# cschin/Peregrine

Measured on AMD Instinct MI355X. Metric: confirmed overlaps/sec (ovlp_t records, index+overlap stages, seqdb resident in HBM), higher is better.
Workload: dtype u8/u32 integer

## Files before the change

### peregrine_amd/csrc/pgx_align.hip

```cpp
#include <hipcub/hipcub.hpp>

#include "pgx_internal.h"

namespace pgx {
namespace {

__device__ __forceinline__ uint64_t load_u64_unaligned(const uint8_t *p) {
  uint64_t v;
  __builtin_memcpy(&v, p, 8);
  return v;
}
struct U128 {
  uint64_t lo, hi;
};
__device__ __forceinline__ U128 load_u128_unaligned(const uint8_t *p) {
  U128 v;
  __builtin_memcpy(&v, p, 16);
  return v;
}
__device__ __forceinline__ int match8(uint64_t qa, uint64_t ta, int qs, int ts) {
  const uint64_t diff = ((qa >> qs) ^ (ta >> ts)) & 0x0F0F0F0F0F0F0F0FULL;
  return diff ? (__builtin_ctzll(diff) >> 3) : 8;
}
__device__ __forceinline__ uint64_t ballot64(bool p) { return __builtin_amdgcn_ballot_w64(p); }
template <int CTRL>
__device__ __forceinline__ int dpp_max(int v) {
  return max(v, __builtin_amdgcn_update_dpp(0, v, CTRL, 0xf, 0xf, true));
}
template <int GL>
__device__ __forceinline__ int group_max_i32(int v) {
  v = dpp_max<0xB1>(v);
  v = dpp_max<0x4E>(v);
  if (GL >= 8) v = dpp_max<0x141>(v);
  if (GL == 16) v = dpp_max<0x140>(v);
  return v;
}
template <int GL>
__device__ __forceinline__ uint32_t group_bits(uint64_t wave_mask, int gbase) {
  return (uint32_t)(wave_mask >> gbase) & ((1u << GL) - 1u);
}
template <int CTRL>
__device__ __forceinline__ int dpp_min(int v) {
  return min(v, __builtin_amdgcn_update_dpp(0, v, CTRL, 0xf, 0xf, true));
}
__device__ __forceinline__ int group_min8_i32(int v) {
  v = dpp_min<0xB1>(v);
  v = dpp_min<0x4E>(v);
  return dpp_min<0x141>(v);
}
__device__ __forceinline__ uint32_t ffbl_or_ones(uint32_t v) {
  uint32_t r;
  asm("v_ffbl_b32 %0, %1" : "=v"(r) : "v"(v));
  return r;
}
__device__ __forceinline__ int group_lane(int v, int gb4, int l) { return __builtin_amdgcn_ds_bpermute(gb4 + (l << 2), v); }

template <int CTRL, int ROW_MASK>
__device__ __forceinline__ int dpp_max_step(int v) {
  return max(v, __builtin_amdgcn_update_dpp(v, v, CTRL, ROW_MASK, 0xf, false));
}
__device__ __forceinline__ int wave_max_i32(int v) {
  v = dpp_max_step<0x111, 0xf>(v);
  v = dpp_max_step<0x112, 0xf>(v);
  v = dpp_max_step<0x114, 0xf>(v);
  v = dpp_max_step<0x118, 0xf>(v);
  v = dpp_max_step<0x142, 0xa>(v);
  v = dpp_max_step<0x143, 0xc>(v);
  return __builtin_amdgcn_readlane(v, 63);
}


}

__device__ __forceinline__ int match16p(const uint8_t *q, uint32_t xq, const uint8_t *t, uint32_t yt) {
  uint2 qd, td;
  __builtin_memcpy(&qd, q + (xq >> 4) * 4, 8), __builtin_memcpy(&td, t + (yt >> 4) * 4, 8);
  const uint32_t df = __builtin_amdgcn_alignbit(qd.y, qd.x, (xq & 15) << 1) ^ __builtin_amdgcn_alignbit(td.y, td.x, (yt & 15) << 1);
  return (int)min(ffbl_or_ones(df) >> 1, 16u);
}
template <bool PACKED>
__device__ __forceinline__ void align_one_per_wave(const uint8_t *__restrict__ seq, const uint64_t *__restrict__ roff,
                                                   const uint32_t *__restrict__ rlen, const pgx_align_key *__restrict__ keys, uint32_t a, int band,
                                                   int ring, pgx_match *__restrict__ out) {
  extern __shared__ int32_t V[];
  constexpr int PB = PACKED ? 16 : 8;
  const int lane = threadIdx.x;
  const pgx_align_key key = keys[a];
  const uint32_t len0 = rlen[key.rid0], len1 = rlen[key.rid1];
  const uint8_t *q = PACKED ? seq + (roff[key.rid0] + (key.dir0 ? (len0 + 15u) >> 4 : 0u) + (key.q_off >> 4)) * 4 : seq + roff[key.rid0] + key.q_off;
  const uint8_t *t = PACKED ? seq + (roff[key.rid1] + (key.dir1 ? (len1 + 15u) >> 4 : 0u)) * 4 : seq + roff[key.rid1];
  const uint32_t qo = PACKED ? key.q_off & 15u : 0u;
  const int q_len = (int)(len0 - key.q_off);
  const int t_len = (int)len1;
  const int qs = key.dir0 ? 4 : 0, ts = key.dir1 ? 4 : 0;
  const int max_d = (int)(0.3 * (double)(q_len + t_len));
  const int band_size = band * 2;
  const int mask = ring - 1;
  for (int i = lane; i < ring; i += 64) V[i] = 0;
  __syncthreads();

  int best_m = -1, min_k = 0, max_k = 0;
  uint32_t longest = 0;
  bool started = false, matched = false;
  int q_bgn = 0, t_bgn = 0, q_m_end = 0, t_m_end = 0, q_end = 0, t_end = 0, dist = 0;

  for (int d = 0; d < max_d; ++d) {
    if (max_k - min_k > band_size) break;
    const int nk = max_k >= min_k ? ((max_k - min_k) >> 1) + 1 : 0;
    int x = 0, y = 0;
    for (int base = 0; base < nk && !matched; base += 64) {
      const int j = base + lane;
      const bool active = j < nk;
      const int k = min_k + 2 * j;
      int x1 = 0, y1 = 0;
      x = 0, y = 0;
      bool more = false;
      if (active) {
        const int va = V[(k - 1) & mask], vb = V[(k + 1) & mask];
        x = (k == min_k || (k != max_k && va < vb)) ? vb : va + 1;
        y = x - k;
        x1 = x, y1 = y;
        const int rem = min(q_len - x, t_len - y);
        if (rem > 0) {
          int m = PACKED ? match16p(q, qo + (uint32_t)x, t, (uint32_t)y) : match8(load_u64_unaligned(q + x), load_u64_unaligned(t + y), qs, ts);
          m = min(m, rem);
          x += m, y += m;
          more = (m == PB) && (rem > PB);
        }
      }
      uint64_t mm = ballot64(more);
      while (mm) {
        const int L = __builtin_ctzll(mm);
        const int xs = __builtin_amdgcn_readlane(x, L), ys = __builtin_amdgcn_readlane(y, L);
        const int rem = min(q_len - xs, t_len - ys);
        const int off = lane * PB;
        int m = 0;
        if (off < rem)
          m = min(PACKED ? match16p(q, qo + (uint32_t)(xs + off), t, (uint32_t)(ys + off))
                         : match8(load_u64_unaligned(q + xs + off), load_u64_unaligned(t + ys + off), qs, ts), rem - off);
        const uint64_t stop = ballot64(m < PB);
        int ext;
        if (stop) {
          const int f = __builtin_ctzll(stop);
          ext = PB * f + __builtin_amdgcn_readlane(m, f);
        } else {
          ext = 64 * PB;
        }
        if (lane == L) x += ext, y += ext;
        if (stop || ext >= rem) mm &= mm - 1;
      }
      const int ext = x - x1;
      const bool hit = active && (x >= q_len || y >= t_len);
      const uint64_t hitmask = ballot64(hit);
      const int hl = hitmask ? __builtin_ctzll(hitmask) : 64;
      const bool valid = active && lane <= hl;
      if (!started) {
        const uint64_t m = ballot64(valid && ext > 16);
        if (m) {
          const int l = __builtin_ctzll(m);
          q_bgn = __builtin_amdgcn_readlane(x1, l), t_bgn = __builtin_amdgcn_readlane(y1, l);
          started = true;
        }
      }
      if (ballot64(valid && (uint32_t)ext > longest)) {
        const int mx = wave_max_i32(valid ? ext : -1);
        const int l = __builtin_ctzll(ballot64(valid && ext == mx));
        longest = (uint32_t)mx;
        q_m_end = __builtin_amdgcn_readlane(x, l), t_m_end = __builtin_amdgcn_readlane(y, l);
      }
      if (valid) V[k & mask] = x;
      best_m = max(best_m, wave_max_i32(valid ? x + y : -1));
      if (hitmask) {
        matched = true;
        q_end = __builtin_amdgcn_readlane(x, hl), t_end = __builtin_amdgcn_readlane(y, hl);
      }
    }
    __syncthreads();
    if (matched) {
      dist = d;
      break;
    }
    int new_min = max_k, new_max = min_k;
    const int thr = best_m - band;
    for (int base = 0; base < nk; base += 64) {
      const int j = base + lane;
      const int k2 = min_k + 2 * j;
      int u;
      if (nk <= 64) u = x + y;
      else u = j < nk ? 2 * V[k2 & mask] - k2 : 0;
      const uint64_t m = ballot64(j < nk && u >= thr);
      if (m) {
        new_min = min(new_min, min_k + 2 * (base + __builtin_ctzll(m)));
        new_max = max(new_max, min_k + 2 * (base + 63 - __builtin_clzll(m)));
      }
    }
    max_k = new_max + 1;
    min_k = new_min - 1;
  }
  if (lane == 0) {
    pgx_match r;
    if (matched) {
      r.q_bgn = q_bgn, r.t_bgn = t_bgn, r.q_end = q_end, r.t_end = t_end, r.dist = dist;
      r.m_size = (q_end - q_bgn + t_end - t_bgn + 2 * dist) / 2;
    } else {
      r.q_bgn = 0, r.t_bgn = 0, r.q_end = 0, r.t_end = 0, r.dist = 0, r.m_size = 0;
    }
    r.q_m_end = q_m_end, r.t_m_end = t_m_end;
    out[a] = r;
  }
}
template <bool PACKED>
__global__ __launch_bounds__(64) void k_align1(const uint8_t *__restrict__ seq, const uint64_t *__restrict__ roff,
                                              const uint32_t *__restrict__ rlen,
                                              const pgx_align_key *__restrict__ keys, uint32_t n, int band,
                                              int ring, pgx_match *__restrict__ out) {
  if (blockIdx.x < n) align_one_per_wave<PACKED>(seq, roff, rlen, keys, blockIdx.x, band, ring, out);
}
template <bool PACKED>
__global__ __launch_bounds__(64) void k_align1_list(const uint8_t *__restrict__ seq, const uint64_t *__restrict__ roff,
                                                   const uint32_t *__restrict__ rlen, const pgx_align_key *__restrict__ keys,
                                                   const uint32_t *__restrict__ list_n, const uint32_t *__restrict__ list, int band, int ring,
                                                   pgx_match *__restrict__ out) {
  const uint32_t cnt = *list_n;
  for (uint32_t i = blockIdx.x; i < cnt; i += gridDim.x) {
    __syncthreads();
    align_one_per_wave<PACKED>(seq, roff, rlen, keys, list[i], band, ring, out);
  }
}


template <int GL, typename VT>
__global__ __launch_bounds__(64) void k_align4(const uint8_t *__restrict__ seq, const uint64_t *__restrict__ roff,
                                               const uint32_t *__restrict__ rlen,
                                               const pgx_align_key *__restrict__ keys, uint32_t n, int band, int ring,
                                               pgx_match *__restrict__ out, uint32_t *__restrict__ counter) {
  extern __shared__ int32_t Vall[];
  const int lane = threadIdx.x, gl = lane & (GL - 1), gbase = lane & ~(GL - 1);
  VT *V = reinterpret_cast<VT *>(Vall) + (lane / GL) * ring;
  const int mask = ring - 1, band_size = band * 2;

  uint32_t c_next = 0, c_end = 0;
  bool alive = false, exhausted = false;
  uint32_t a = 0;
  const uint8_t *q = seq, *t = seq;
  int q_len = 0, t_len = 0, qs = 0, ts = 0, max_d = 0, d = 0;
  int best_m = -1, min_k = 0, max_k = 0;
  uint32_t longest = 0;
  bool started = false, matched = false;
  int q_bgn = 0, t_bgn = 0, q_m_end = 0, t_m_end = 0, q_end = 0, t_end = 0;

  for (;;) {
    const bool fetching = !alive && !exhausted;
    const uint64_t fw = ballot64(fetching);
    uint32_t na = 0;
    if (fw) {
      constexpr uint32_t CHUNK = 8;
      uint64_t need = 0;
      for (int g = 0; g < 64; g += GL) need |= 1ULL << g;
      need &= fw;
      const uint32_t cnt = (uint32_t)__builtin_popcountll(need);
      const uint32_t r = __builtin_amdgcn_mbcnt_hi((uint32_t)(need >> 32), __builtin_amdgcn_mbcnt_lo((uint32_t)need, 0u));
      const uint32_t avail = __builtin_amdgcn_readfirstlane(c_end - c_next);
      na = c_next + r;
      if (avail < cnt) {
        uint32_t got = 0;
        if (lane == 0) got = atomicAdd(counter, CHUNK);
        got = __builtin_amdgcn_readfirstlane(got);
        if (r >= avail) na = got + (r - avail);
        c_next = got + (cnt - avail), c_end = got + CHUNK;
      } else {
        c_next += cnt;
      }
    }
    if (fetching) {
      na = (uint32_t)__shfl((int)na, gbase, 64);
      if (na >= n) {
        exhausted = true;
      } else {
        a = na;
        const pgx_align_key key = keys[a];
        q = seq + roff[key.rid0] + key.q_off;
        t = seq + roff[key.rid1];
        q_len = (int)(rlen[key.rid0] - key.q_off);
        t_len = (int)rlen[key.rid1];
        qs = key.dir0 ? 4 : 0, ts = key.dir1 ? 4 : 0;
        max_d = (int)(0.3 * (double)(q_len + t_len));
        d = 0, best_m = -1, min_k = 0, max_k = 0, longest = 0;
        started = matched = false;
        q_bgn = t_bgn = q_m_end = t_m_end = q_end = t_end = 0;
        if (gl == 0) V[1 & mask] = (VT)0;
        alive = true;
      }
    }
    if (!ballot64(alive)) break;
    __syncthreads();

    bool stepping = alive;
    if (alive && (d >= max_d || max_k - min_k > band_size)) {
      if (gl == 0) {
        pgx_match r;
        r.m_size = 0, r.dist = 0, r.q_bgn = 0, r.q_end = 0, r.t_bgn = 0, r.t_end = 0;
        r.t_m_end = t_m_end, r.q_m_end = q_m_end;
        out[a] = r;
      }
      alive = false, stepping = false;
    }

    const int nk = max_k >= min_k ? ((max_k - min_k) >> 1) + 1 : 0;
    int x = 0, y = 0;
    for (int base = 0;; base += GL) {
      const bool inround = stepping && !matched && base < nk;
      if (!ballot64(inround)) break;
      const int j = base + gl;
      const bool active = inround && j < nk;
      const int k = min_k + 2 * j;
      int x1 = 0, y1 = 0;
      bool more = false;
      if (inround) x = 0, y = 0;
      if (active) {
        const int va = (int)V[(k - 1) & mask], vb = (int)V[(k + 1) & mask];
        x = (k == min_k || (k != max_k && va < vb)) ? vb : va + 1;
        y = x - k;
        x1 = x, y1 = y;
        const int rem = min(q_len - x, t_len - y);
        if (rem > 0) {
          int m = match8(load_u64_unaligned(q + x), load_u64_unaligned(t + y), qs, ts);
          m = min(m, rem);
          x += m, y += m;
          more = (m == 8) && (rem > 8);
        }
      }
      uint64_t mw = ballot64(more);
      while (mw) {
        const uint32_t gm = group_bits<GL>(mw, gbase);
        const bool has = gm != 0;
        const int L = has ? __builtin_ctz(gm) : 0;
        const int xs = __shfl(x, gbase + L, 64), ys = __shfl(y, gbase + L, 64);
        const int rem = min(q_len - xs, t_len - ys);
        constexpr int SL = GL == 16 ? 8 : 16;
        const int off = gl * SL;
        int m = SL;
        if (has) {
          m = 0;
          if (off < rem) {
            m = match8(load_u64_unaligned(q + xs + off), load_u64_unaligned(t + ys + off), qs, ts);
            if (SL == 16 && m == 8 && off + 8 < rem)
              m += match8(load_u64_unaligned(q + xs + off + 8), load_u64_unaligned(t + ys + off + 8), qs, ts);
            m = min(m, rem - off);
          }
        }
        const uint32_t sg = group_bits<GL>(ballot64(has && m < SL), gbase);
        int ext = GL * SL;
        if (sg) {
          const int f = __builtin_ctz(sg);
          ext = SL * f + __shfl(m, gbase + f, 64);
        }
        if (has && gl == L) {
          x += ext, y += ext;
          if (sg || ext >= rem) more = false;
        }
        mw = ballot64(more);
      }
      const int ext = x - x1;
      const bool hit = active && (x >= q_len || y >= t_len);
      const uint64_t hitw = ballot64(hit);
      int hl = GL;
      if (hitw) {
        const uint32_t hitm = group_bits<GL>(hitw, gbase);
        if (hitm) hl = __builtin_ctz(hitm);
      }
      const bool valid = active && gl <= hl;
      {
        const uint64_t sw = ballot64(valid && ext > 16 && !started);
        if (sw) {
          const uint32_t m = group_bits<GL>(sw, gbase);
          const int l = m ? __builtin_ctz(m) : 0;
          const int bx = __shfl(x1, gbase + l, 64), by = __shfl(y1, gbase + l, 64);
          if (m) q_bgn = bx, t_bgn = by, started = true;
        }
      }
      if (ballot64(valid && (uint32_t)ext > longest)) {
        const int mx = group_max_i32<GL>(valid ? ext : -1);
        const uint32_t m = group_bits<GL>(ballot64(valid && ext == mx), gbase);
        const int l = m ? __builtin_ctz(m) : 0;
        const int ex = __shfl(x, gbase + l, 64), ey = __shfl(y, gbase + l, 64);
        if (inround && mx >= 0 && (uint32_t)mx > longest) longest = (uint32_t)mx, q_m_end = ex, t_m_end = ey;
      }
      if (valid) V[k & mask] = (VT)x;
      {
        const int s = group_max_i32<GL>(valid ? x + y : -1);
        if (inround) best_m = max(best_m, s);
      }
      if (hitw) {
        const uint32_t hitm = group_bits<GL>(hitw, gbase);
        const int ex = __shfl(x, gbase + (hl & (GL - 1)), 64), ey = __shfl(y, gbase + (hl & (GL - 1)), 64);
        if (inround && hitm) matched = true, q_end = ex, t_end = ey;
      }
    }
    __syncthreads();

    if (stepping && matched) {
      if (gl == 0) {
        pgx_match r;
        r.q_bgn = q_bgn, r.t_bgn = t_bgn, r.q_end = q_end, r.t_end = t_end, r.dist = d;
        r.m_size = (q_end - q_bgn + t_end - t_bgn + 2 * d) / 2;
        r.t_m_end = t_m_end, r.q_m_end = q_m_end;
        out[a] = r;
      }
      alive = false, stepping = false;
    }
    int new_min = max_k, new_max = min_k;
    const int thr = best_m - band;
    for (int base = 0;; base += GL) {
      const bool inround = stepping && base < nk;
      if (!ballot64(inround)) break;
      const int j = base + gl;
      const int k2 = min_k + 2 * j;
      int u = 0;
      if (inround && j < nk) u = (nk <= GL) ? x + y : 2 * (int)V[k2 & mask] - k2;
      const uint32_t m = group_bits<GL>(ballot64(inround && j < nk && u >= thr), gbase);
      if (m) {
        new_min = min(new_min, min_k + 2 * (base + __builtin_ctz(m)));
        new_max = max(new_max, min_k + 2 * (base + 31 - __builtin_clz(m)));
      }
    }
    if (stepping) max_k = new_max + 1, min_k = new_min - 1, ++d;
  }
}


enum { PH_FETCH = 0, PH_STEP = 1, PH_ROUND = 2, PH_SNAKE = 3, PH_END = 4, PH_BAND = 5, PH_DONE = 6 };
#ifdef PGX_PH_BARRIER
#define PH_SYNC() __syncthreads()
#else
#define PH_SYNC() __builtin_amdgcn_fence(__ATOMIC_RELEASE, "wavefront"), __builtin_amdgcn_fence(__ATOMIC_ACQUIRE, "wavefront")
#endif
template <int GL, typename VT, bool PACKED>
__global__ __launch_bounds__(1024, 8) void k_align_ph(const uint8_t *__restrict__ seq, const uint64_t *__restrict__ roff,
                                                      const uint32_t *__restrict__ rlen, const pgx_align_key *__restrict__ keys,
                                                      uint32_t n, int band, int ring, pgx_match *__restrict__ out,
                                                      uint32_t *__restrict__ counter, const uint32_t *__restrict__ redo_n,
                                                      const uint32_t *__restrict__ redo_list, uint32_t *__restrict__ esc_n,
                                                      uint32_t *__restrict__ esc_list, const uint32_t *__restrict__ nflag, uint32_t seg,
                                                      uint32_t iter_limit) {
  extern __shared__ int32_t Vall[];
  __shared__ unsigned long long s_state;
  __shared__ uint32_t s_lock;
  static_assert(GL == 8, "the group operations below are written for 8-lane groups (half a DPP row)");
  const int lane = threadIdx.x & 63, gl = lane & (GL - 1), gbase = lane & ~(GL - 1), gb4 = gbase << 2;
  VT *V = reinterpret_cast<VT *>(Vall) + ((threadIdx.x >> 6) * (64 / GL) + lane / GL) * ring;
  if (threadIdx.x == 0) s_state = (unsigned long long)seg, s_lock = 0u;
  __syncthreads();
  const int mask = ring - 1, band_size = band * 2;
  constexpr int SL = PACKED ? 32 : (GL == 16 ? 8 : 16);
  constexpr int PROBE = PACKED ? 16 : 8;
  if (redo_list) n = *redo_n;
  const uint32_t iter_budget = esc_list && iter_limit ? iter_limit : 0xFFFFFFFFu;
  uint32_t qo = 0, to = 0;
  uint32_t iters = 0;
  uint32_t c_next = 0, c_end = 0;

  int phase = PH_FETCH;
  uint32_t a = 0;
  const uint8_t *q = seq, *t = seq;
  int q_len = 0, t_len = 0, qs = 0, ts = 0, max_d = 0, d = 0;
  int best_m = -1, min_k = 0, max_k = 0, nk = 0, base = 0, bbase = 0, new_min = 0, new_max = 0;
  uint32_t longest = 0;
  bool started = false;
  int q_bgn = 0, t_bgn = 0, q_m_end = 0, t_m_end = 0;
  int x = 0, y = 0, x1 = 0, y1 = 0, k = 0;
  bool active = false;
  uint32_t gm = 0;

#ifdef PGX_ALIGN_STATS
  uint32_t my_iters = 0;
  int my_maxnk = 0;
  bool has_cand = false;
#endif
  for (;;) {
#ifdef PGX_ALIGN_STATS
    if (phase == PH_FETCH && has_cand && gl == 0 && !redo_list) {
      const uint32_t b = my_iters ? 31u - (uint32_t)__builtin_clz(my_iters) : 0u;
      atomicAdd(counter + 1 + min(b, 31u), 1u);
#ifdef PGX_ALIGN_STATS_NK
      atomicAdd(counter + 33 + min((uint32_t)my_maxnk, 31u), 1u);
#else
      atomicAdd(counter + 33 + min(b, 31u), my_iters);
#endif
    }
    if (phase == PH_FETCH) has_cand = false, my_iters = 0, my_maxnk = 0;
    my_maxnk = max(my_maxnk, phase == PH_ROUND || phase == PH_STEP ? nk : 0);
    ++my_iters;
#endif
    ++iters;
    constexpr uint32_t RETRY = 0xFFFFFFFFu;
    const bool fetching = phase == PH_FETCH;
    const uint64_t fw = ballot64(fetching);
    uint32_t na = 0;
    if (fw) {
      constexpr uint32_t CHUNK = 8;
      const uint64_t need = fw & 0x0101010101010101ULL;
      const uint32_t cnt = (uint32_t)__builtin_popcountll(need);
      const uint32_t r = __builtin_amdgcn_mbcnt_hi((uint32_t)(need >> 32), __builtin_amdgcn_mbcnt_lo((uint32_t)need, 0u));
      const uint32_t avail = __builtin_amdgcn_readfirstlane(c_end - c_next);
      na = c_next + r;
      if (avail < cnt) {
        uint32_t got = RETRY;
        if (lane == 0) {
          unsigned long long o = atomicAdd(&s_state, (unsigned long long)CHUNK);
          if ((uint32_t)o < seg) {
            got = (uint32_t)(o >> 32) + (uint32_t)o;
          } else if (atomicCAS(&s_lock, 0u, 1u) == 0u) {
            o = atomicAdd(&s_state, (unsigned long long)CHUNK);
            if ((uint32_t)o < seg) {
              got = (uint32_t)(o >> 32) + (uint32_t)o;
            } else {
              got = atomicAdd(counter, seg);
              atomicExch(&s_state, ((unsigned long long)got << 32) | CHUNK);
            }
            atomicExch(&s_lock, 0u);
          }
        }
        got = __builtin_amdgcn_readfirstlane(got);
        if (got == RETRY) {
          if (r >= avail) na = RETRY;
          c_next = c_end = 0;
        } else {
          if (r >= avail) na = got + (r - avail);
          c_next = got + (cnt - avail), c_end = got + CHUNK;
        }
      } else {
        c_next += cnt;
      }
    }
    if (fetching) {
      iters = 0;
      na = (uint32_t)group_lane((int)na, gb4, 0);
      if (na == RETRY) {
      } else if (na >= n) {
        phase = PH_DONE;
      } else {
#ifdef PGX_ALIGN_STATS
        has_cand = true;
#endif
        a = redo_list ? redo_list[na] : na;
        const pgx_align_key key = keys[a];
        const uint32_t len0 = rlen[key.rid0], len1 = rlen[key.rid1];
        if (PACKED) {
          q = seq + (roff[key.rid0] + (key.dir0 ? (len0 + 15u) >> 4 : 0u) + (key.q_off >> 4)) * 4;
          t = seq + (roff[key.rid1] + (key.dir1 ? (len1 + 15u) >> 4 : 0u)) * 4;
          qo = key.q_off & 15u, to = 0;
        } else {
          q = seq + roff[key.rid0] + key.q_off;
          t = seq + roff[key.rid1];
        }
        q_len = (int)(len0 - key.q_off);
        t_len = (int)len1;
        qs = key.dir0 ? 4 : 0, ts = key.dir1 ? 4 : 0;
        max_d = (int)(0.3 * (double)(q_len + t_len));
        d = 0, best_m = -1, min_k = 0, max_k = 0, longest = 0;
        started = false;
        q_bgn = t_bgn = q_m_end = t_m_end = 0;
        if (gl == 0) V[1 & mask] = (VT)0;
        phase = PH_STEP;
        if (PACKED && ((nflag[key.rid0] | nflag[key.rid1]) & 1u)) {
          if (gl == 0) esc_list[n + atomicAdd(esc_n + 1, 1u)] = a;
          phase = PH_FETCH;
        }
      }
    }
    if (!ballot64(phase != PH_DONE)) break;
    PH_SYNC();

    if (iters > iter_budget && phase == PH_STEP && !(d >= max_d || max_k - min_k > band_size)) {
      if (gl == 0) esc_list[atomicAdd(esc_n, 1u)] = a;
      phase = PH_FETCH;
    }
    if (phase == PH_STEP) {
      const int width = max_k - min_k;
      if (d >= max_d || width > band_size) {
        if (gl == 0) {
          pgx_match r;
          r.m_size = 0, r.dist = 0, r.q_bgn = 0, r.q_end = 0, r.t_bgn = 0, r.t_end = 0;
          r.t_m_end = t_m_end, r.q_m_end = q_m_end;
          out[a] = r;
        }
        phase = PH_FETCH;
      } else if (width < 0) {
        nk = 0, base = 0, bbase = 0, new_min = max_k, new_max = min_k, phase = PH_BAND;
      } else {
        nk = (width >> 1) + 1, base = 0, phase = PH_ROUND;
      }
    }

    int probe_full = 0;
    if (phase == PH_ROUND) {
      const int j = base + gl;
      active = j < nk;
      k = min_k + 2 * j;
      if (active) {
        const int va = (int)V[(k - 1) & mask], vb = (int)V[(k + 1) & mask];
        x = (k == min_k || (k != max_k && va < vb)) ? vb : va + 1;
        y = x - k;
        x1 = x, y1 = y;
        const int rem = min(q_len - x, t_len - y);
        if (rem > 0) {
          int m;
          if (PACKED) {
            const uint32_t xq = qo + (uint32_t)x, yt = to + (uint32_t)y;
            uint2 qd, td;
            __builtin_memcpy(&qd, q + (xq >> 4) * 4, 8), __builtin_memcpy(&td, t + (yt >> 4) * 4, 8);
            const uint32_t df = __builtin_amdgcn_alignbit(qd.y, qd.x, (xq & 15) << 1) ^ __builtin_amdgcn_alignbit(td.y, td.x, (yt & 15) << 1);
            m = (int)min(ffbl_or_ones(df) >> 1, 16u);
          } else {
            m = match8(load_u64_unaligned(q + x), load_u64_unaligned(t + y), qs, ts);
          }
          probe_full = (int)min((uint32_t)m, (uint32_t)(rem - 1));
          m = (int)min((uint32_t)m, (uint32_t)rem);
          x += m, y += m;
        }
      }
    }
    {
      asm volatile("" : "+v"(probe_full));
      const uint32_t g = group_bits<GL>(ballot64(probe_full >= PROBE), gbase);
      if (phase == PH_ROUND) gm = g, phase = g ? PH_SNAKE : PH_END;
    }

    {
      const bool sn = phase == PH_SNAKE;
      if (ballot64(sn)) {
        const int L = __builtin_ctz(gm | 0x100u);
        const int xs = group_lane(x, gb4, L), ys = group_lane(y, gb4, L);
        const int rem = min(q_len - xs, t_len - ys);
        const int off = gl * SL;
        int e = GL * SL;
        if (sn) {
          e = off;
          if (off < rem) {
            int m;
            if (PACKED) {
              const uint32_t xq = qo + (uint32_t)(xs + off), yt = to + (uint32_t)(ys + off);
              uint4 qd, td;
              __builtin_memcpy(&qd, q + (xq >> 4) * 4, 16), __builtin_memcpy(&td, t + (yt >> 4) * 4, 16);
              const uint32_t qsh = (xq & 15) << 1, tsh = (yt & 15) << 1;
              const uint32_t d0 = __builtin_amdgcn_alignbit(qd.y, qd.x, qsh) ^ __builtin_amdgcn_alignbit(td.y, td.x, tsh);
              const uint32_t d1 = __builtin_amdgcn_alignbit(qd.z, qd.y, qsh) ^ __builtin_amdgcn_alignbit(td.z, td.y, tsh);
              m = (int)min(min(ffbl_or_ones(d0), ffbl_or_ones(d1) | 32u) >> 1, 32u);
            } else {
              const U128 qa = load_u128_unaligned(q + xs + off), ta = load_u128_unaligned(t + ys + off);
              m = match8(qa.lo, ta.lo, qs, ts);
              if (m == 8) m += match8(qa.hi, ta.hi, qs, ts);
            }
            m = (int)min((uint32_t)m, (uint32_t)(rem - off));
            e = m < SL ? off + m : GL * SL;
          }
        }
        const int ext = group_min8_i32(e);
        if (sn) {
          if (gl == L) x += ext, y += ext;
          if (ext < GL * SL || ext >= rem) gm &= gm - 1;
          if (!gm) phase = PH_END;
        }
      }
    }

    {
      const bool e = phase == PH_END;
      const int ext = x - x1;
      const bool hit = e && active && (x >= q_len || y >= t_len);
      const uint64_t hitw = ballot64(hit);
      int hl = GL;
      uint32_t hitm = 0;
      if (hitw) {
        hitm = group_bits<GL>(hitw, gbase);
        if (hitm) hl = __builtin_ctz(hitm);
        asm volatile("" : "+v"(hl));
      }
      const bool valid = e && active && gl <= hl;
      {
        const uint64_t sw = ballot64((valid && !started ? ext : 0) > 16);
        if (sw) {
          const uint32_t m = group_bits<GL>(sw, gbase);
          const int l = m ? __builtin_ctz(m) : 0;
          const int bx = group_lane(x1, gb4, l), by = group_lane(y1, gb4, l);
          if (m) q_bgn = bx, t_bgn = by, started = true;
        }
      }
      const int ev = valid ? ext : -1;
      if (ballot64(ev > (int)longest)) {
        const int mx = group_max_i32<GL>(ev);
        const uint32_t m = group_bits<GL>(ballot64(valid && ext == mx), gbase);
        const int l = m ? __builtin_ctz(m) : 0;
        const int ex = group_lane(x, gb4, l), ey = group_lane(y, gb4, l);
        if (e && mx >= 0 && (uint32_t)mx > longest) longest = (uint32_t)mx, q_m_end = ex, t_m_end = ey;
      }
      if (valid) V[k & mask] = (VT)x;
      const int u = x + y;
      {
        const int s = group_max_i32<GL>(valid ? u : -1);
        if (e) best_m = max(best_m, s);
      }
      bool matched = false;
      if (hitw) {
        const int ex = group_lane(x, gb4, hl & (GL - 1)), ey = group_lane(y, gb4, hl & (GL - 1));
        if (e && hitm) {
          matched = true;
          if (gl == 0) {
            pgx_match r;
            r.q_bgn = q_bgn, r.t_bgn = t_bgn, r.q_end = ex, r.t_end = ey, r.dist = d;
            r.m_size = (ex - q_bgn + ey - t_bgn + 2 * d) / 2;
            r.t_m_end = t_m_end, r.q_m_end = q_m_end;
            out[a] = r;
          }
        }
      }
      const uint32_t qm = group_bits<GL>(ballot64((e && active ? u : INT32_MIN) >= best_m - band), gbase);
      if (e) {
        if (matched) {
          phase = PH_FETCH;
        } else if (nk <= GL) {
          const int lo = qm ? min_k + 2 * __builtin_ctz(qm) : max_k, hi = qm ? min_k + 2 * (31 - __builtin_clz(qm)) : min_k;
          max_k = hi + 1, min_k = lo - 1, ++d, phase = PH_STEP;
        } else {
          base += GL;
          phase = PH_ROUND;
          if (base >= nk) bbase = 0, new_min = max_k, new_max = min_k, phase = PH_BAND;
        }
      }
    }
    PH_SYNC();

    {
      const bool bnd = phase == PH_BAND;
      if (ballot64(bnd)) {
        const int thr = best_m - band;
        const int j = bbase + gl;
        const int k2 = min_k + 2 * j;
        int u = 0;
        if (bnd && j < nk) u = 2 * (int)V[k2 & mask] - k2;
        const uint32_t m = group_bits<GL>(ballot64((bnd && j < nk ? u : INT32_MIN) >= thr), gbase);
        if (bnd) {
          if (m) {
            new_min = min(new_min, min_k + 2 * (bbase + __builtin_ctz(m)));
            new_max = max(new_max, min_k + 2 * (bbase + 31 - __builtin_clz(m)));
          }
          bbase += GL;
          if (bbase >= nk) max_k = new_max + 1, min_k = new_min - 1, ++d, phase = PH_STEP;
        }
      }
    }
  }
}

__global__ void k_order_keys(const pgx_align_key *__restrict__ keys, uint32_t n, const uint32_t *__restrict__ prank, uint32_t *__restrict__ k,
                             uint32_t *__restrict__ v, uint32_t *__restrict__ n_out) {
  const uint32_t i = blockIdx.x * blockDim.x + threadIdx.x;
  if (i == 0) *n_out = n;
  if (i < n) k[i] = prank[keys[i].rid0], v[i] = i;
}

void dev_align_prepare(const pgx_seqdb *db) {
  const char *pm = getenv("PGX_ALIGN_PACKED_MIN");
  if (db->max_rlen > 65535u || (pm && atol(pm) < 0)) return;
  (void)seq_packs(db);
}

void dev_align(const pgx_seqdb *db, const pgx_align_key *d_keys, size_t n, int band, pgx_match *d_out, int tail_batch) {
  if (n == 0) return;
  const long small_max = getenv("PGX_ALIGN_SMALL") ? atol(getenv("PGX_ALIGN_SMALL")) : tail_batch >= 2 ? 250000 : tail_batch ? 60000 : 13000;
  KernelTimer tm((long)n <= small_max ? "align1" : "align", n);
  int ring = 64;
  while (ring < 2 * band + 8) ring <<= 1;
  hipStream_t st = ctx().stream;
  const bool one_packed = seq_packs_valid(db) && db->n_flagged_reads == 0 && db->max_rlen <= 65535u &&
                          (!db->d_seq.p || !(getenv("PGX_ALIGN1_PACKED") && atoi(getenv("PGX_ALIGN1_PACKED")) == 0));
  PGX_REQUIRE(db->d_seq.p || one_packed, PGX_ESTATE, "the seqdb's bytes were released (pgx_seqdb_release_bytes) and its packs are gone");
  if ((long)n <= small_max) {
    if (one_packed)
      hipLaunchKernelGGL(k_align1<true>, dim3((unsigned)n), dim3(64), ring * sizeof(int32_t), st, reinterpret_cast<const uint8_t *>(db->d_pack.p), db->d_poff.p,
                         db->d_rlen.p, d_keys, (uint32_t)n, band, ring, d_out);
    else
      hipLaunchKernelGGL(k_align1<false>, dim3((unsigned)n), dim3(64), ring * sizeof(int32_t), st, db->d_seq.p, db->d_roff.p, db->d_rlen.p, d_keys,
                         (uint32_t)n, band, ring, d_out);
    PGX_HIP(hipGetLastError());
    return;
  }
  uint32_t *counter = ws<uint32_t>("align.counter", 8);
  PGX_HIP(hipMemsetAsync(counter, 0, 8 * sizeof(uint32_t), st));
  if (db->max_rlen > 65535u) {
    const unsigned grid = (unsigned)std::min<size_t>((n + 7) / 8, (size_t)ctx().num_cu * 20);
    hipLaunchKernelGGL((k_align4<8, int32_t>), dim3(grid), dim3(64), 8 * ring * sizeof(int32_t), st, db->d_seq.p, db->d_roff.p, db->d_rlen.p,
                       d_keys, (uint32_t)n, band, ring, d_out, counter);
    PGX_HIP(hipGetLastError());
    return;
  }
  const size_t lds_wave = (size_t)8 * ring * sizeof(uint16_t);
  const unsigned waves_cu = (unsigned)std::min<size_t>(32, (158u << 10) / lds_wave);
  const long nw_env = getenv("PGX_ALIGN_NW") ? atol(getenv("PGX_ALIGN_NW")) : 0;
  unsigned NW = 1;
  for (unsigned c = 16; c >= 1; c >>= 1)
    if (c <= waves_cu && (waves_cu / c) * c > (waves_cu / NW) * NW) NW = c;
  if (waves_cu >= 16 && (waves_cu / 16) * 16 >= (waves_cu / NW) * NW) NW = 16;
  if (nw_env >= 1 && nw_env <= 16 && (unsigned)nw_env <= waves_cu) NW = (unsigned)nw_env;
  const size_t lds = lds_wave * NW;
  const unsigned wg_cu = waves_cu / NW;
  const char *pm = getenv("PGX_ALIGN_PACKED_MIN");
  const long packed_min = pm ? atol(pm) : 100000;
  const uint32_t *packs = (packed_min >= 0 && ((long)n >= packed_min || seq_packs_valid(db))) ? seq_packs(db) : nullptr;
  const size_t n_wg = (size_t)ctx().num_cu * wg_cu;
  auto segment = [&](size_t cnt) {
    const long se = getenv("PGX_ALIGN_SEG") ? atol(getenv("PGX_ALIGN_SEG")) : 0;
    size_t sg = se > 0 ? (size_t)se : std::min<size_t>(512, std::max<size_t>(8 * NW, cnt / (n_wg * 16)));
    return (uint32_t)((sg + 7) & ~(size_t)7);
  };
  const uint32_t seg = segment(n);
  const unsigned grid = (unsigned)std::min<size_t>((n + seg - 1) / seg, n_wg);
  if (packs) {
    const uint32_t iter_limit = getenv("PGX_ALIGN_ITER_LIMIT") ? (uint32_t)atol(getenv("PGX_ALIGN_ITER_LIMIT")) : 2500u;
    uint32_t *esc = ws<uint32_t>("align.esc", 2 * n + 4);
    PGX_HIP(hipMemsetAsync(esc, 0, 3 * sizeof(uint32_t), st));
    const uint32_t *order = nullptr;
    const long order_min = getenv("PGX_ALIGN_ORDER_MIN") ? atol(getenv("PGX_ALIGN_ORDER_MIN")) : 200000;
    if (db->locus_ordered && order_min >= 0 && (long)n >= order_min) {
      const uint32_t nn = (uint32_t)n;
      uint32_t *k_in = ws<uint32_t>("align.ord_kin", n), *k_out = ws<uint32_t>("align.ord_kout", n), *v_in = ws<uint32_t>("align.ord_vin", n),
               *v_out = ws<uint32_t>("align.ord_vout", n);
      hipLaunchKernelGGL(k_order_keys, dim3((nn + 255) / 256), dim3(256), 0, st, d_keys, nn, db->d_prank.p, k_in, v_in, esc + 3);
      int bits = 1;
      while (bits < 32 && (db->rlen_by_rid.size() >> bits)) ++bits;
      size_t tb = 0;
      PGX_HIP(hipcub::DeviceRadixSort::SortPairs(nullptr, tb, k_in, k_out, v_in, v_out, (int)nn, 0, bits, st));
      void *tmp = ws_raw("align.ord_tmp", tb + 256);
      PGX_HIP(hipcub::DeviceRadixSort::SortPairs(tmp, tb, k_in, k_out, v_in, v_out, (int)nn, 0, bits, st));
      order = v_out;
    }
    hipLaunchKernelGGL((k_align_ph<8, uint16_t, true>), dim3(grid), dim3(64 * NW), lds, st, reinterpret_cast<const uint8_t *>(packs), db->d_poff.p,
                       db->d_rlen.p, d_keys, (uint32_t)n, band, ring, d_out, counter, order ? esc + 3 : (const uint32_t *)nullptr, order, esc,
                       esc + 4, db->d_nflag.p, seg, iter_limit);
    if (db->n_flagged_reads) {
      const uint32_t seg2 = segment(n / 16 + 1);
      hipLaunchKernelGGL((k_align_ph<8, uint16_t, false>), dim3((unsigned)std::min<size_t>(n / (64 * NW) + 8, n_wg)), dim3(64 * NW), lds, st,
                         db->d_seq.p, db->d_roff.p, db->d_rlen.p, d_keys, (uint32_t)n, band, ring, d_out, esc + 2, esc + 1, esc + 4 + n, esc, esc + 4,
                         (const uint32_t *)nullptr, seg2, iter_limit);
    }
    const dim3 g1((unsigned)std::min<size_t>(std::max<size_t>(n / 256, 256), (size_t)ctx().num_cu * 32));
    if (one_packed)
      hipLaunchKernelGGL(k_align1_list<true>, g1, dim3(64), ring * sizeof(int32_t), st, reinterpret_cast<const uint8_t *>(packs), db->d_poff.p, db->d_rlen.p,
                         d_keys, esc, esc + 4, band, ring, d_out);
    else
      hipLaunchKernelGGL(k_align1_list<false>, g1, dim3(64), ring * sizeof(int32_t), st, db->d_seq.p, db->d_roff.p, db->d_rlen.p, d_keys, esc, esc + 4, band,
                         ring, d_out);
  } else {
    hipLaunchKernelGGL((k_align_ph<8, uint16_t, false>), dim3(grid), dim3(64 * NW), lds, st, db->d_seq.p, db->d_roff.p, db->d_rlen.p, d_keys,
                       (uint32_t)n, band, ring, d_out, counter, (const uint32_t *)nullptr, (const uint32_t *)nullptr, (uint32_t *)nullptr,
                       (uint32_t *)nullptr, (const uint32_t *)nullptr, seg, 0u);
  }
  PGX_HIP(hipGetLastError());
}

}
```

Baseline: 61.45 million.

## Add fast path for narrow-band wave iterations in phased aligner kernel

Adds a FAST template variant of the phased alignment kernel. When every lane group in a wavefront is in the STEP phase with a diagonal band narrow enough to fit one 8-lane group (or is done), it runs step, probe, snake and end-of-round in a single loop iteration. This skips the separate STEP→ROUND→SNAKE→END phase transitions and their intermediate syncs. It is enabled by default, can be turned off with an environment variable, and adds optional stats counters. The cost is extra code and register pressure, plus a wave-wide ballot check on every iteration.

```diff
diff --git a/peregrine_amd/csrc/pgx_align.hip b/peregrine_amd/csrc/pgx_align.hip
--- a/peregrine_amd/csrc/pgx_align.hip
+++ b/peregrine_amd/csrc/pgx_align.hip
@@ -1,4 +1,6 @@
 #include <hipcub/hipcub.hpp>
+
+#include <type_traits>
 
 #include "pgx_internal.h"
 
@@ -435,7 +437,7 @@
 #else
 #define PH_SYNC() __builtin_amdgcn_fence(__ATOMIC_RELEASE, "wavefront"), __builtin_amdgcn_fence(__ATOMIC_ACQUIRE, "wavefront")
 #endif
-template <int GL, typename VT, bool PACKED>
+template <int GL, typename VT, bool PACKED, bool FAST>
 __global__ __launch_bounds__(1024, 8) void k_align_ph(const uint8_t *__restrict__ seq, const uint64_t *__restrict__ roff,
                                                       const uint32_t *__restrict__ rlen, const pgx_align_key *__restrict__ keys,
                                                       uint32_t n, int band, int ring, pgx_match *__restrict__ out,
@@ -476,6 +478,7 @@
   uint32_t my_iters = 0;
   int my_maxnk = 0;
   bool has_cand = false;
+  uint64_t st_iters = 0, st_fast = 0, st_fast_ext0 = 0, st_fast_ext1 = 0;
 #endif
   for (;;) {
 #ifdef PGX_ALIGN_STATS
@@ -572,32 +575,8 @@
     if (!ballot64(phase != PH_DONE)) break;
     PH_SYNC();
 
-    if (iters > iter_budget && phase == PH_STEP && !(d >= max_d || max_k - min_k > band_size)) {
-      if (gl == 0) esc_list[atomicAdd(esc_n, 1u)] = a;
-      phase = PH_FETCH;
-    }
-    if (phase == PH_STEP) {
-      const int width = max_k - min_k;
-      if (d >= max_d || width > band_size) {
-        if (gl == 0) {
-          pgx_match r;
-          r.m_size = 0, r.dist = 0, r.q_bgn = 0, r.q_end = 0, r.t_bgn = 0, r.t_end = 0;
-          r.t_m_end = t_m_end, r.q_m_end = q_m_end;
-          out[a] = r;
-        }
-        phase = PH_FETCH;
-      } else if (width < 0) {
-        nk = 0, base = 0, bbase = 0, new_min = max_k, new_max = min_k, phase = PH_BAND;
-      } else {
-        nk = (width >> 1) + 1, base = 0, phase = PH_ROUND;
-      }
-    }
-
-    int probe_full = 0;
-    if (phase == PH_ROUND) {
-      const int j = base + gl;
-      active = j < nk;
-      k = min_k + 2 * j;
+    auto round_probe = [&]() -> int {
+      int probe_full = 0;
       if (active) {
         const int va = (int)V[(k - 1) & mask], vb = (int)V[(k + 1) & mask];
         x = (k == min_k || (k != max_k && va < vb)) ? vb : va + 1;
@@ -620,14 +599,11 @@
           x += m, y += m;
         }
       }
-    }
-    {
       asm volatile("" : "+v"(probe_full));
-      const uint32_t g = group_bits<GL>(ballot64(probe_full >= PROBE), gbase);
-      if (phase == PH_ROUND) gm = g, phase = g ? PH_SNAKE : PH_END;
-    }
-
-    {
+      return probe_full;
+    };
+
+    auto snake = [&]() {
       const bool sn = phase == PH_SNAKE;
       if (ballot64(sn)) {
         const int L = __builtin_ctz(gm | 0x100u);
@@ -663,9 +639,10 @@
           if (!gm) phase = PH_END;
         }
       }
-    }
-
-    {
+    };
+
+    auto end_round = [&](auto one_round) {
+      constexpr bool ONE_ROUND = decltype(one_round)::value;
       const bool e = phase == PH_END;
       const int ext = x - x1;
       const bool hit = e && active && (x >= q_len || y >= t_len);
@@ -719,7 +696,7 @@
       if (e) {
         if (matched) {
           phase = PH_FETCH;
-        } else if (nk <= GL) {
+        } else if (ONE_ROUND || nk <= GL) {
           const int lo = qm ? min_k + 2 * __builtin_ctz(qm) : max_k, hi = qm ? min_k + 2 * (31 - __builtin_clz(qm)) : min_k;
           max_k = hi + 1, min_k = lo - 1, ++d, phase = PH_STEP;
         } else {
@@ -728,7 +705,74 @@
           if (base >= nk) bbase = 0, new_min = max_k, new_max = min_k, phase = PH_BAND;
         }
       }
-    }
+    };
+
+    if (FAST) {
+      const int width = max_k - min_k;
+      const bool live = phase == PH_STEP;
+      const bool qual = phase == PH_DONE ||
+                        (live && iters <= iter_budget && d < max_d && (uint32_t)width <= (uint32_t)min(band_size, 2 * (GL - 1)));
+      const bool go = !ballot64(!qual);
+#ifdef PGX_ALIGN_STATS
+      ++st_iters;
+      if (go) ++st_fast;
+#endif
+      if (go) {
+        nk = (width >> 1) + 1, base = 0;
+        k = min_k + 2 * gl;
+        active = live && gl < nk;
+        gm = group_bits<GL>(ballot64(round_probe() >= PROBE), gbase);
+        if (live) phase = gm ? PH_SNAKE : PH_END;
+#ifdef PGX_ALIGN_STATS
+        if (!ballot64(gm != 0u)) ++st_fast_ext0;
+#endif
+        snake();
+#ifdef PGX_ALIGN_STATS
+        if (!ballot64(phase == PH_SNAKE)) ++st_fast_ext1;
+#endif
+        end_round(std::true_type());
+        PH_SYNC();
+        continue;
+      }
+    }
+
+    if (iters > iter_budget && phase == PH_STEP && !(d >= max_d || max_k - min_k > band_size)) {
+      if (gl == 0) esc_list[atomicAdd(esc_n, 1u)] = a;
+      phase = PH_FETCH;
+    }
+    if (phase == PH_STEP) {
+      const int width = max_k - min_k;
+      if (d >= max_d || width > band_size) {
+        if (gl == 0) {
+          pgx_match r;
+          r.m_size = 0, r.dist = 0, r.q_bgn = 0, r.q_end = 0, r.t_bgn = 0, r.t_end = 0;
+          r.t_m_end = t_m_end, r.q_m_end = q_m_end;
+          out[a] = r;
+        }
+        phase = PH_FETCH;
+      } else if (width < 0) {
+        nk = 0, base = 0, bbase = 0, new_min = max_k, new_max = min_k, phase = PH_BAND;
+      } else {
+        nk = (width >> 1) + 1, base = 0, phase = PH_ROUND;
+      }
+    }
+
+    int probe_full = 0;
+    if (phase == PH_ROUND) {
+      const int j = base + gl;
+      active = j < nk;
+      k = min_k + 2 * j;
+      probe_full = round_probe();
+    }
+    {
+      asm volatile("" : "+v"(probe_full));
+      const uint32_t g = group_bits<GL>(ballot64(probe_full >= PROBE), gbase);
+      if (phase == PH_ROUND) gm = g, phase = g ? PH_SNAKE : PH_END;
+    }
+
+    snake();
+
+    end_round(std::false_type());
     PH_SYNC();
 
     {
@@ -751,6 +795,13 @@
       }
     }
   }
+#ifdef PGX_ALIGN_STATS
+  if (lane == 0 && (nflag || !esc_list)) {
+    unsigned long long *st = reinterpret_cast<unsigned long long *>(counter + 72);
+    atomicAdd(st + 0, (unsigned long long)st_iters), atomicAdd(st + 1, (unsigned long long)st_fast);
+    atomicAdd(st + 2, (unsigned long long)st_fast_ext0), atomicAdd(st + 3, (unsigned long long)st_fast_ext1);
+  }
+#endif
 }
 
 __global__ void k_order_keys(const pgx_align_key *__restrict__ keys, uint32_t n, const uint32_t *__restrict__ prank, uint32_t *__restrict__ k,
@@ -786,8 +837,13 @@
     PGX_HIP(hipGetLastError());
     return;
   }
-  uint32_t *counter = ws<uint32_t>("align.counter", 8);
-  PGX_HIP(hipMemsetAsync(counter, 0, 8 * sizeof(uint32_t), st));
+#ifdef PGX_ALIGN_STATS
+  constexpr size_t n_counter = 80;
+#else
+  constexpr size_t n_counter = 8;
+#endif
+  uint32_t *counter = ws<uint32_t>("align.counter", n_counter);
+  PGX_HIP(hipMemsetAsync(counter, 0, n_counter * sizeof(uint32_t), st));
   if (db->max_rlen > 65535u) {
     const unsigned grid = (unsigned)std::min<size_t>((n + 7) / 8, (size_t)ctx().num_cu * 20);
     hipLaunchKernelGGL((k_align4<8, int32_t>), dim3(grid), dim3(64), 8 * ring * sizeof(int32_t), st, db->d_seq.p, db->d_roff.p, db->d_rlen.p,
@@ -795,6 +851,7 @@
     PGX_HIP(hipGetLastError());
     return;
   }
+  const bool fast = !(getenv("PGX_ALIGN_FAST") && atoi(getenv("PGX_ALIGN_FAST")) == 0);
   const size_t lds_wave = (size_t)8 * ring * sizeof(uint16_t);
   const unsigned waves_cu = (unsigned)std::min<size_t>(32, (158u << 10) / lds_wave);
   const long nw_env = getenv("PGX_ALIGN_NW") ? atol(getenv("PGX_ALIGN_NW")) : 0;
@@ -835,12 +892,23 @@
       PGX_HIP(hipcub::DeviceRadixSort::SortPairs(tmp, tb, k_in, k_out, v_in, v_out, (int)nn, 0, bits, st));
       order = v_out;
     }
-    hipLaunchKernelGGL((k_align_ph<8, uint16_t, true>), dim3(grid), dim3(64 * NW), lds, st, reinterpret_cast<const uint8_t *>(packs), db->d_poff.p,
-                       db->d_rlen.p, d_keys, (uint32_t)n, band, ring, d_out, counter, order ? esc + 3 : (const uint32_t *)nullptr, order, esc,
-                       esc + 4, db->d_nflag.p, seg, iter_limit);
+    hipLaunchKernelGGL((fast ? k_align_ph<8, uint16_t, true, true> : k_align_ph<8, uint16_t, true, false>), dim3(grid), dim3(64 * NW), lds, st,
+                       reinterpret_cast<const uint8_t *>(packs), db->d_poff.p, db->d_rlen.p, d_keys, (uint32_t)n, band, ring, d_out, counter,
+                       order ? esc + 3 : (const uint32_t *)nullptr, order, esc, esc + 4, db->d_nflag.p, seg, iter_limit);
+#ifdef PGX_ALIGN_STATS
+    {
+      uint64_t h[4];
+      PGX_HIP(hipMemcpyAsync(h, counter + 72, sizeof h, hipMemcpyDeviceToHost, st));
+      PGX_HIP(hipStreamSynchronize(st));
+      fprintf(stderr, "[pgx] align stats: n %zu fast %d wave_iters %llu fast_iters %llu (%.2f %%) no_ext %llu (%.2f %%) at_most_one_ext %llu (%.2f %%)\n", n,
+              (int)fast, (unsigned long long)h[0], (unsigned long long)h[1], 100.0 * (double)h[1] / (double)(h[0] ? h[0] : 1), (unsigned long long)h[2],
+              100.0 * (double)h[2] / (double)(h[0] ? h[0] : 1), (unsigned long long)h[3], 100.0 * (double)h[3] / (double)(h[0] ? h[0] : 1));
+    }
+#endif
     if (db->n_flagged_reads) {
       const uint32_t seg2 = segment(n / 16 + 1);
-      hipLaunchKernelGGL((k_align_ph<8, uint16_t, false>), dim3((unsigned)std::min<size_t>(n / (64 * NW) + 8, n_wg)), dim3(64 * NW), lds, st,
+      hipLaunchKernelGGL((fast ? k_align_ph<8, uint16_t, false, true> : k_align_ph<8, uint16_t, false, false>),
+                         dim3((unsigned)std::min<size_t>(n / (64 * NW) + 8, n_wg)), dim3(64 * NW), lds, st,
                          db->d_seq.p, db->d_roff.p, db->d_rlen.p, d_keys, (uint32_t)n, band, ring, d_out, esc + 2, esc + 1, esc + 4 + n, esc, esc + 4,
                          (const uint32_t *)nullptr, seg2, iter_limit);
     }
@@ -852,7 +920,8 @@
       hipLaunchKernelGGL(k_align1_list<false>, g1, dim3(64), ring * sizeof(int32_t), st, db->d_seq.p, db->d_roff.p, db->d_rlen.p, d_keys, esc, esc + 4, band,
                          ring, d_out);
   } else {
-    hipLaunchKernelGGL((k_align_ph<8, uint16_t, false>), dim3(grid), dim3(64 * NW), lds, st, db->d_seq.p, db->d_roff.p, db->d_rlen.p, d_keys,
+    hipLaunchKernelGGL((fast ? k_align_ph<8, uint16_t, false, true> : k_align_ph<8, uint16_t, false, false>), dim3(grid), dim3(64 * NW), lds, st,
+                       db->d_seq.p, db->d_roff.p, db->d_rlen.p, d_keys,
                        (uint32_t)n, band, ring, d_out, counter, (const uint32_t *)nullptr, (const uint32_t *)nullptr, (uint32_t *)nullptr,
                        (uint32_t *)nullptr, (const uint32_t *)nullptr, seg, 0u);
   }
```

After: 61.29 million, median of 3. No clear change (-0.3%).
